# KIT-MBS/pydca

Hardware: AMD Instinct MI355X
Metric: plmDCA L-BFGS iterations/s (L=500 N=50000 q=21) (higher is better)
Workload: dtype f32

## Files before the change

### pydca_amd/csrc/lbfgs_kernels.h

```cpp
#pragma once

#include "dca_internal.h"
#include "plm_plan.h"
#include "vec_kernels.h"

namespace {

template <bool DD> struct DotAcc;
template <> struct DotAcc<false> {
    double hi = 0.0;
    static constexpr double lo = 0.0;
    __device__ __forceinline__ void add(double a, double b) { hi += a * b; }
    __device__ __forceinline__ void wave_reduce() { for (int off = 32; off > 0; off >>= 1) hi += __shfl_down(hi, off); }
};
template <> struct DotAcc<true> {
    double hi = 0.0, lo = 0.0;
    __device__ __forceinline__ void add(double a, double b) { dd_add(hi, lo, __dmul_rn(a, b)); }
    __device__ __forceinline__ void wave_reduce() { dd_wave_reduce(hi, lo); }
};
template <int NV>
__device__ __forceinline__ void dot_block_store(double (*red)[2 * NV], int nv, double* __restrict__ partials, unsigned grid = 0)
{
    __syncthreads();
    if ((int)threadIdx.x < nv) {
// ... 91 lines not shown
        Pack<T> pse; Pack<T> pye;
        _Pragma("unroll") for (int u = 0; u < VEC; ++u) {
            pse.v[u] = px.v[u] - pxp.v[u]; pye.v[u] = pg.v[u] - pgp.v[u];
            acc[0].add((double)pye.v[u], (double)pse.v[u]); acc[1].add((double)pye.v[u], (double)pye.v[u]);
        }
        psk[E] = pse; pyk[E] = pye;
        stp(se, iv, pse); stp(ye, iv, pye);
        _Pragma("unroll") for (int k = 0; k < 5; ++k) {
            _Pragma("unroll") for (int u = 0; u < VEC; ++u) {
                const double gv = pg.v[u]; const double sev = pse.v[u]; const double yev = pye.v[u];
                const double sk = psk[k].v[u]; const double yk = pyk[k].v[u];
                acc[2 + k].add(sk, gv); acc[7 + k].add(yk, gv); acc[12 + k].add(sev, yk); acc[17 + k].add(yev, sk); acc[22 + k].add(yev, yk);
            }
        },
        { const T sev_ = x[i] - xp[i]; const T yev_ = g[i] - gp[i]; se[i] = sev_; ye[i] = yev_;
          const double gv = g[i]; const double sev = sev_; const double yev = yev_;
          acc[0].add(yev, sev); acc[1].add(yev, yev);
          _Pragma("unroll") for (int k = 0; k < 5; ++k) {
              const double sk = k == E ? sev : (double)static_cast<const T*>(P.s[k])[i]; const double yk = k == E ? yev : (double)static_cast<const T*>(P.y[k])[i];
              acc[2 + k].add(sk, gv); acc[7 + k].add(yk, gv); acc[12 + k].add(sev, yk); acc[17 + k].add(yev, sk); acc[22 + k].add(yev, yk);
          } })
    const int lane = threadIdx.x & 63, wv = threadIdx.x >> 6;
#pragma unroll
    for (int v = 0; v < 27; ++v) {
        acc[v].wave_reduce();
        if (lane == 0) { red[wv][2 * v] = acc[v].hi; red[wv][2 * v + 1] = acc[v].lo; }
    }
    dot_block_store<27>(red, 27, partials);
}

template <typename T>
__global__ void vec_compose_kernel(T* __restrict__ d, const T* __restrict__ g, VecPtrs5 P, const DirCoefs* __restrict__ cp, size_t n)
{
    const DirCoefs c = *cp;
    DCA_VEC_LOOP(n, d,
        const Pack<T> pg = ldp(g, iv);
        double v[VEC];
        _Pragma("unroll") for (int u = 0; u < VEC; ++u) v[u] = c.g * (double)pg.v[u];
        _Pragma("unroll") for (int k = 0; k < 5; ++k) {
            const Pack<T> psk = ldp(static_cast<const T*>(P.s[k]), iv); const Pack<T> pyk = ldp(static_cast<const T*>(P.y[k]), iv);
            _Pragma("unroll") for (int u = 0; u < VEC; ++u) v[u] += c.s[k] * (double)psk.v[u] + c.y[k] * (double)pyk.v[u];
        }
        Pack<T> o;
        _Pragma("unroll") for (int u = 0; u < VEC; ++u) o.v[u] = (T)v[u];
        stp(d, iv, o);,
        { double v = c.g * (double)g[i];
          _Pragma("unroll") for (int k = 0; k < 5; ++k)
              v += c.s[k] * (double)static_cast<const T*>(P.s[k])[i] + c.y[k] * (double)static_cast<const T*>(P.y[k])[i];
          d[i] = (T)v; })
}
#undef ldp
#undef stp

__global__ __launch_bounds__(256)
void vec_final_kernel(const double* __restrict__ partials, int nb, int nk, double* __restrict__ out)
{
    __shared__ double redHi[256], redLo[256];
    const int k = blockIdx.x;
    double hi = 0.0, lo = 0.0;
    for (int b = threadIdx.x; b < nb; b += blockDim.x) dd_add2(hi, lo, partials[2 * ((size_t)k * nb + b)], partials[2 * ((size_t)k * nb + b) + 1]);
    dd_block_reduce(hi, lo, redHi, redLo);
    if (threadIdx.x == 0) out[k] = hi + lo;
}

__global__ __launch_bounds__(256)
void dd_sum_chunks_kernel(const double* __restrict__ parts, int n, double* __restrict__ out)
{
    __shared__ double redHi[256], redLo[256];
    const int chunk = (n + gridDim.x - 1) / gridDim.x;
    const int lo_ = blockIdx.x * chunk, hi_ = min(n, lo_ + chunk);
    double hi = 0.0, lo = 0.0;
    for (int b = lo_ + threadIdx.x; b < hi_; b += blockDim.x) dd_add2(hi, lo, parts[2 * (size_t)b], parts[2 * (size_t)b + 1]);
    dd_block_reduce(hi, lo, redHi, redLo);
    if (threadIdx.x == 0) { out[2 * blockIdx.x] = hi; out[2 * blockIdx.x + 1] = lo; }
}
__global__ __launch_bounds__(1024)
void dd_sum_final_kernel(const double* __restrict__ A, int nA, const double* __restrict__ B, int nB, double* __restrict__ out)
{
    __shared__ double redHi[1024], redLo[1024];
    double hi = 0.0, lo = 0.0;
    for (int b = threadIdx.x; b < nA; b += blockDim.x) dd_add2(hi, lo, A[2 * (size_t)b], A[2 * (size_t)b + 1]);
    for (int b = threadIdx.x; b < nB; b += blockDim.x) dd_add2(hi, lo, B[2 * (size_t)b], B[2 * (size_t)b + 1]);
    dd_block_reduce(hi, lo, redHi, redLo);
    if (threadIdx.x == 0) out[0] = hi + lo;
}

template <typename T>
__global__ __launch_bounds__(kVecThreads)
void vec_dot3_fx_kernel(const T* __restrict__ a, const T* __restrict__ b, const T* __restrict__ c, size_t n, double* __restrict__ partials,
                        const double* __restrict__ fxParts, int nFxParts, double* __restrict__ fxChunks)
{
    if (blockIdx.x >= (unsigned)kVecBlocks) {
        __shared__ double redHi[256], redLo[256];
        const int blk = (int)blockIdx.x - kVecBlocks;
        const int chunk = (nFxParts + kSumStageBlocks - 1) / kSumStageBlocks;
        const int lo_ = blk * chunk, hi_ = min(nFxParts, lo_ + chunk);
        double hi = 0.0, lo = 0.0;
        for (int p = lo_ + threadIdx.x; p < hi_; p += blockDim.x) dd_add2(hi, lo, fxParts[2 * (size_t)p], fxParts[2 * (size_t)p + 1]);
        dd_block_reduce(hi, lo, redHi, redLo);
        if (threadIdx.x == 0) { fxChunks[2 * blk] = hi; fxChunks[2 * blk + 1] = lo; }
        return;
    }
    __shared__ double red[kVecThreads / 64][6];
    DotAcc<sizeof(T) == 8> s0, s1, s2;
    DCA_VEC_LOOP_G(n, a, kVecBlocks,
        const Pack<T> pa = ldp_at(a + head_, iv); const Pack<T> pb = ldp_at(b + head_, iv); const Pack<T> pc = ldp_at(c + head_, iv);
// ... 42 lines not shown
```

### pydca_amd/csrc/plm_engine.hip

```cpp
#include <algorithm>
#include <chrono>
#include <cmath>

#include "dca_internal.h"
#include "more_thuente.h"
#include "vec_kernels.h"
#include "plm_plan.h"
#include "plm_stages.h"
#include "lbfgs_kernels.h"

namespace {

static_assert(kPlanXcds == kNumXcd, "the planner deals strips to this many XCDs");

#ifdef DCA_ROUND_ABLATE
__global__ void round_to_f32_kernel(double* __restrict__ p, size_t n)
{
    for (size_t i = blockIdx.x * (size_t)blockDim.x + threadIdx.x; i < n; i += (size_t)gridDim.x * blockDim.x) p[i] = (double)(float)p[i];
}
inline int round_stage_mask() { const char* e = getenv("DCA_ROUND_F32_STAGES"); return e ? atoi(e) : 0; }
#define DCA_ROUND_STAGE(bit, ptr, count)                                                                             \
    do {                                                                                                             \
        if constexpr (sizeof(T) == 8)                                                                                \
            if (round_stage_mask() & (bit))                                                                          \
// ... 1 lines not shown
    } while (0)
#else
#define DCA_ROUND_STAGE(bit, ptr, count) do { } while (0)
#endif

template <typename T>
struct PlmEngine : PlmEngineBase {
    dca_ctx* ctx;
    int N, L, q, Ls;
    double lambda_h = 0, lambda_J = 0;
    int carry_mode = DCA_CARRY_CHUNKED, halo = 0, add_reg = 1;
    bool configured = false;
    PlmPlan plan;
    PlmKnobs knobs;

    T *dx = nullptr, *dg = nullptr, *dxp = nullptr, *dgp = nullptr, *dd = nullptr;
    T* dS[5] = {nullptr, nullptr, nullptr, nullptr, nullptr};
    T* dY[5] = {nullptr, nullptr, nullptr, nullptr, nullptr};
    T *dWt = nullptr, *dSR = nullptr, *dR = nullptr, *dG = nullptr, *dw = nullptr;
    LbfgsDev* dLb = nullptr;
    uint16_t* dXL = nullptr;
    uint16_t* dXT2 = nullptr;
    PairIJ* dPairs = nullptr;
    double *dFxPart = nullptr, *dRegPart = nullptr, *dVecPart = nullptr;
    double *dColPart = nullptr, *dColSum = nullptr;
    double* dColChunk = nullptr;
    bool stripRequested = false, strips = false, stripEmulate = false;
    int sWorld = 1, sRank = 0;
    T *dGrecv = nullptr, *dXsend = nullptr, *dXrecv = nullptr;
    template <typename F> void each_buffer(F f)
    {
        f(dx); f(dg); f(dxp); f(dgp); f(dd);
        for (int i = 0; i < 5; ++i) { f(dS[i]); f(dY[i]); }
        f(dWt); f(dSR); f(dR); f(dG); f(dw); f(dLb); f(dXL); f(dXT2); f(dPairs); f(dFxPart); f(dRegPart); f(dVecPart);
        f(dColPart); f(dColSum); f(dColChunk); f(dGrecv); f(dXsend); f(dXrecv);
    }
    int strip_cs(int r) const { return plm_strip_cs(plan.siteB, q, r); }
    size_t owned_lo(int r) const { return plm_owned_lo(plan.siteB, L, q, r); }
    size_t owned_hi(int r) const { return plm_owned_hi(plan.siteB, L, q, r); }
    bool lbfgs_alloc = false;
    bool deferFx = false, fxPending = false;
    size_t vlo = 0, vn = 0, Ppad = 0;
    dca_comm_hook comm = nullptr;
    void* comm_user = nullptr;
    int comm_rank = 0, comm_world = 0;

    struct {
        bool begun = false, finished = false;
        int status = 0, k = 1, end = 0, iters = 0, evals = 0, max_iterations = 0, verbose = 0;
        double fx = 0, step = 0, xnorm = 0, gnorm = 0, seconds = 0;
        double last_step = 0;
        double dginit = 0;
        bool dginit_on_device = false;
    } o;

    explicit PlmEngine(dca_ctx* c) : ctx(c), N(c->N), L(c->L), q(c->q), Ls(c->Ls) {}

    template <typename U> int dalloc(U** p, size_t n)
    {
        HIP_TRY(dca_dev_malloc(reinterpret_cast<void**>(p), std::max<size_t>(n, 1) * sizeof(U)));
        return DCA_OK;
    }
    void freeall() { each_buffer([](auto*& p) { dca_dev_free(p); p = nullptr; }); }
    ~PlmEngine() override { freeall(); }

    void weights_changed() override { configured = false; o = decltype(o)(); }

    int configure(double lh, double lJ, int cmode, int chunk_, int warm_, int halo_, int add_reg_) override
    {
        if (q != 21 && q != 5) { dca_set_error("plmDCA kernels are built for q = 21 (protein) and q = 5 (RNA); got %d", q); return DCA_ERR_ARG; }
        if (!ctx->have_weights) { dca_set_error("weights must be computed or set before dca_plm_configure"); return DCA_ERR_STATE; }
        if (halo_ < 0 || halo_ >= N) { dca_set_error("halo out of range"); return DCA_ERR_ARG; }
        if (L > 65535) { dca_set_error("L too large"); return DCA_ERR_ARG; }
        configured = false;
        lambda_h = lh; lambda_J = lJ; carry_mode = cmode; halo = halo_; add_reg = add_reg_;
        strips = stripRequested && ctx->comm && ctx->comm_world > 1;
        stripRequested = false;
        sWorld = strips ? ctx->comm_world : 1;
        sRank = strips ? ctx->comm_rank : 0;
#ifdef DCA_ROUND_ABLATE
        stripEmulate = false;
        if (const char* e = getenv("DCA_STRIP_EMULATE")) {
            int er = 0, ew = 1;
            if (sscanf(e, "%d,%d", &er, &ew) == 2 && ew > 1 && er >= 0 && er < ew) { strips = true; stripEmulate = true; sRank = er; sWorld = ew; }
        }
#endif
        if (sWorld > kMaxStripRanks || (strips && sWorld > L)) { dca_set_error("column strips: too many ranks for %d sites", L); return DCA_ERR_ARG; }
        if (strips && (halo || hook || comm)) { dca_set_error("column strips take the whole alignment and no hooks"); return DCA_ERR_ARG; }
        knobs = PlmKnobs::from_env();
        PlmShape shape;
        shape.N = N; shape.L = L; shape.q = q; shape.elemBytes = (int)sizeof(T); shape.halo = halo; shape.chunkArg = chunk_; shape.warmArg = warm_;
        shape.carryMode = carry_mode; shape.stripWorld = sWorld; shape.stripRank = sRank; shape.strips = strips;
        plan = plm_make_plan(shape, knobs, PlmKernelShapes{{logits_seq_per_wg(5), logits_seq_per_wg(21), logits_seq_per_wg(kPairQ)},
                                                           {logits_jt(5), logits_jt(21), logits_jt(kPairQ)}});
        const int Lq = L * q, JT = plan.JT;
        const size_t npairs = (size_t)L * (L - 1) / 2;

        freeall();
        lbfgs_alloc = false;
        o = decltype(o)();

        DCA_TRY(dalloc(&dx, plan.P + kVecPad)); DCA_TRY(dalloc(&dg, plan.P + kVecPad));
        DCA_TRY(dalloc(&dWt, (size_t)plan.Wrows * plan.Cs));
        DCA_TRY(dalloc(&dSR, (size_t)N * plan.Cs));
        DCA_TRY(dalloc(&dR, (size_t)(N + kNC) * plan.Cs));
        HIP_TRY(hipMemsetAsync(dR, 0, (size_t)(N + kNC) * plan.Cs * sizeof(T), ctx->stream));
// ... 59 lines not shown
            hipLaunchKernelGGL(plm_build_pair_states_kernel, dim3(ceil_div(plan.Npad, 256), ceil_div(plan.gUnits, JT) * JT), dim3(256), 0,
                               ctx->stream, ctx->dX, dXL, N, plan.Npad, L, Ls, 0, 0x2000u);
            hipLaunchKernelGGL(plm_build_pair_states_kernel, dim3(ceil_div(plan.NT, 256), plan.gUnits), dim3(256), 0, ctx->stream,
                               ctx->dX, dXT2, N, plan.NT, L, Ls, halo, 0x9000u);
            HIP_TRY(hipGetLastError());
            HIP_TRY(hipStreamSynchronize(ctx->stream));
        } else {
            hipLaunchKernelGGL(plm_build_logit_states_kernel, dim3(ceil_div(plan.Npad, 256), ceil_div(L, JT) * JT), dim3(256), 0,
                               ctx->stream, ctx->dX, dXL, N, plan.Npad, L, Ls);
            hipLaunchKernelGGL(plm_build_states_kernel, dim3(ceil_div(plan.NT, 256), L), dim3(256), 0, ctx->stream,
                               ctx->dX, dXT2, N, L, Ls, halo, plan.NT);
            HIP_TRY(hipGetLastError());
            HIP_TRY(hipStreamSynchronize(ctx->stream));
        }
        configured = true;
        return DCA_OK;
    }

    int configure_strips(double lh, double lJ, int cmode, int chunk_, int warm_) override
    {
        if (!ctx->comm) { dca_set_error("column strips need a communicator: dca_comm_init first"); return DCA_ERR_STATE; }
        if (o.begun && !o.finished) { dca_set_error("the decomposition cannot change during an optimisation"); return DCA_ERR_STATE; }
        const auto hook0 = hook; const auto hookUser0 = hook_user; const auto comm0 = comm; const auto commUser0 = comm_user;
        const int commRank0 = comm_rank, commWorld0 = comm_world;
        hook = nullptr; hook_user = nullptr; comm = nullptr; comm_user = nullptr; comm_rank = comm_world = 0;
        stripRequested = true;
        const int rc = configure(lh, lJ, cmode, chunk_, warm_, 0, 1);
        stripRequested = false;
        if (rc != DCA_OK) { hook = hook0; hook_user = hookUser0; comm = comm0; comm_user = commUser0; comm_rank = commRank0; comm_world = commWorld0; strips = false; }
        return rc;
    }

    int init_x() override
    {
        if (!configured) { dca_set_error("dca_plm_configure first"); return DCA_ERR_STATE; }
        std::vector<T> hw(N);
        HIP_TRY(hipMemcpy(hw.data(), dw, (size_t)N * sizeof(T), hipMemcpyDeviceToHost));
        T meff = 0;
        for (int n = 0; n < N; ++n) meff += hw[n];
        std::vector<T> h((size_t)L * q, (T)0);
        const uint8_t* X = dca_host_msa(ctx);
        if (!X) return DCA_ERR_HIP;
        for (int n = 0; n < N; ++n)
            for (int i = 0; i < L; ++i) h[(size_t)i * q + X[(size_t)n * L + i]] += hw[n];
        for (int i = 0; i < L; ++i) {
            T* hi = h.data() + (size_t)i * q;
            for (int a = 0; a < q; ++a) hi[a] /= meff;
            for (int a = 0; a < q; ++a) hi[a] = std::log(hi[a] * meff + (T)1);
            T s = 0;
            for (int a = 0; a < q; ++a) s += hi[a];
            const T av = s / (T)q;
            for (int a = 0; a < q; ++a) hi[a] -= av;
        }
        HIP_TRY(hipMemsetAsync(dx, 0, plan.P * sizeof(T), ctx->stream));
        HIP_TRY(hipMemcpyAsync(dx, h.data(), h.size() * sizeof(T), hipMemcpyHostToDevice, ctx->stream));
        HIP_TRY(hipStreamSynchronize(ctx->stream));
        return DCA_OK;
    }

    template <typename U> int upload(const U* src, T* dst)
    {
        std::vector<T> tmp(plan.P);
        for (size_t i = 0; i < plan.P; ++i) tmp[i] = (T)src[i];
        HIP_TRY(hipMemcpy(dst, tmp.data(), plan.P * sizeof(T), hipMemcpyHostToDevice));
        return DCA_OK;
    }
    template <typename U> int download(const T* src, U* dst)
    {
        std::vector<T> tmp(plan.P);
        HIP_TRY(hipStreamSynchronize(ctx->stream));
        HIP_TRY(hipMemcpy(tmp.data(), src, plan.P * sizeof(T), hipMemcpyDeviceToHost));
        for (size_t i = 0; i < plan.P; ++i) dst[i] = (U)tmp[i];
        return DCA_OK;
    }
    int set_x(const void* x, int dtype) override
    {
        if (!configured) { dca_set_error("dca_plm_configure first"); return DCA_ERR_STATE; }
        if (dtype == DCA_F32) return upload(static_cast<const float*>(x), dx);
        if (dtype == DCA_F64) return upload(static_cast<const double*>(x), dx);
        return DCA_ERR_ARG;
    }
    int get_x(void* x, int dtype) override
    {
        if (!configured) return DCA_ERR_STATE;
        if (native_mode == 4 && !stripEmulate) DCA_TRY(strip_allgather(dx));
        if (dtype == DCA_F32) return download(dx, static_cast<float*>(x));
        if (dtype == DCA_F64) return download(dx, static_cast<double*>(x));
        return DCA_ERR_ARG;
    }
    int get_g(void* g, int dtype) override
    {
        if (!configured) return DCA_ERR_STATE;
        DCA_TRY(gather_vector(dg));
        if (dtype == DCA_F32) return download(dg, static_cast<float*>(g));
        if (dtype == DCA_F64) return download(dg, static_cast<double*>(g));
        return DCA_ERR_ARG;
    }

    template <int Q> int launch_eval()
    {
        hipStream_t st = ctx->stream;
        const size_t npairs = (size_t)L * (L - 1) / 2;
        {
            ScopedKernelClock kc(ctx, "plm_expand");
            hipLaunchKernelGGL(plm_expand_kernel<T>, dim3((unsigned)npairs), dim3(256), (size_t)q * q * sizeof(T), st,
                               dx, dWt, dPairs, L, q, plan.Cs, plan.cS0, plan.cS1);
        }
        DCA_ROUND_STAGE(1, dWt, (size_t)plan.Wrows * plan.Cs);
        {
            const int numCT = plan.numCT;
            auto launch = [&](auto kern, int QL) -> int {
                const int numNB = plan.Npad / logits_seq_per_wg(QL);
                const int blocks = numCT * numNB;
                const size_t lds = (size_t)2 * 128 * 512 + (size_t)logits_waves(QL) * 256;
                HIP_TRY(hipFuncSetAttribute(reinterpret_cast<const void*>(kern), hipFuncAttributeMaxDynamicSharedMemorySize, (int)lds));
                ScopedKernelClock kc(ctx, "plm_logits");
                hipLaunchKernelGGL(kern, dim3(blocks), dim3(logits_waves(QL) * 64), lds, st, dWt, dXL, dSR, N, plan.Npad, plan.gUnits, plan.Cs, numCT, numNB);
                return DCA_OK;
            };
            bool done = false;
            if constexpr (Q == 5 && sizeof(T) == 4) {
                if (plan.pairs) {
                    if (plan.pairJT == 11) DCA_TRY(launch(plm_logits_kernel<T, kPairQ, 11>, kPairQ));
                    else if (plan.pairJT == 10) DCA_TRY(launch(plm_logits_kernel<T, kPairQ, 10>, kPairQ));
                    else DCA_TRY(launch(plm_logits_kernel<T, kPairQ>, kPairQ));
                    done = true;
                }
            }
            if (!done) DCA_TRY(launch(plm_logits_kernel<T, Q>, Q));
        }
        DCA_ROUND_STAGE(2, dSR, (size_t)N * plan.Cs);
        {
            dim3 grid(ceil_div(plan.Lloc, 64), ceil_div(plan.numScanChunks, 4));
            ScopedKernelClock kc(ctx, "plm_softmax");
            constexpr int softNP = (64 * Q * (int)sizeof(T) + 1023) / 1024;
            const size_t softLds = (size_t)4 * 2 * softNP * 1024;
            HIP_TRY(hipFuncSetAttribute(reinterpret_cast<const void*>(plm_softmax_kernel<T, Q>), hipFuncAttributeMaxDynamicSharedMemorySize, (int)softLds));
            hipLaunchKernelGGL((plm_softmax_kernel<T, Q>), grid, dim3(256), softLds, st, dSR, dR, dx + (size_t)plan.cS0 * q, ctx->dX + plan.cS0, dw, dFxPart,
                               N, plan.Lloc, Ls, plan.Cs, halo, plan.chunk, plan.warm, carry_mode != DCA_CARRY_EXACT ? 1 : 0, plan.numScanChunks, dColChunk);
        }
        DCA_ROUND_STAGE(4, dR, (size_t)N * plan.Cs);
        {
            const size_t lds = (size_t)2 * kNC * kRowBytes;
            const ScatterStage& sc = plan.scatter;
            auto launch = [&](auto kern) -> int {
                HIP_TRY(hipFuncSetAttribute(reinterpret_cast<const void*>(kern), hipFuncAttributeMaxDynamicSharedMemorySize, (int)lds));
                ScopedKernelClock kc(ctx, "plm_scatter");
                for (int i = 0; i < sc.numLaunches; ++i) {
                    const ScatterLaunch& a = sc.launch[i];
                    hipLaunchKernelGGL(kern, dim3(a.gridX, a.gridY), dim3(sc.threads), lds, st, dR, dXT2, dG,
                                       a.N, a.L, a.Cs, a.halo, a.numChunks, a.NT, a.ctBase, a.numPairs, a.splitX, a.numJG, a.chunksPerSplit, a.slabElems, a.blockChunks,
                                       a.firstBlocksX, a.ctBase2, a.numPairs2, a.splitX2, a.chunksPerSplit2);
                }
                if (sc.sumRemCols)
                    hipLaunchKernelGGL(plm_sum_slabs_cols_kernel<T>, dim3(sc.colsGrid), dim3(256), 0, st, dG,
                                       plan.slab_elems(), plan.Cs, sc.col0, sc.ncols, sc.colRows, sc.colSplit, sc.colZero);
// ... 4 lines not shown
                else if (plan.scatWaves == 4) DCA_TRY(launch(plm_scatter_kernel<T, Q, 2, 4>));
                else DCA_TRY(launch(plm_scatter_kernel<T, Q, 2, 16>));
            } else if constexpr (Q == 5) {
                if (plan.pairs) DCA_TRY(launch(plm_scatter_kernel<T, kPairQ, 2, 16>));
                else DCA_TRY(launch(plm_scatter_kernel<T, Q, 2, 16>));
            } else {
                DCA_TRY(launch(plm_scatter_kernel<T, Q, 2, 16>));
            }
        }
        DCA_ROUND_STAGE(8, dG, plan.num_slabs() * plan.slab_elems());
        {
            ScopedKernelClock kc(ctx, "plm_fold");
            const int LqLoc = plan.Lloc * q;
            int foldSlabs = plan.scatSplit;
            if (plan.scatSplit > 2 || (strips && plan.scatSplit > 1)) {
                hipLaunchKernelGGL(plm_sum_slabs_kernel<T>, dim3(2048), dim3(256), 0, st, dG, plan.slab_elems(), plan.scatSplit);
                foldSlabs = 1;
            }
            if (dColSum) {
                if (dColChunk)
                    hipLaunchKernelGGL(plm_colsum_chunks_kernel, dim3(ceil_div(LqLoc, 256), kColSumRowBlocks), dim3(256), 0, st, dColChunk, plan.numScanChunks, LqLoc, dColPart);
                else
                    hipLaunchKernelGGL(plm_colsum_parts_kernel<T>, dim3(ceil_div(LqLoc, 64), kColSumRowBlocks), dim3(256), 0, st, dR, N, plan.Cs, LqLoc, dColPart);
                hipLaunchKernelGGL(plm_colsum_final_kernel, dim3(ceil_div(LqLoc, 256)), dim3(256), 0, st, dColPart, kColSumRowBlocks, LqLoc, dColSum);
            }
            const int nOwned = plan.pairEnd - plan.pairBegin;
            const bool mergeFields = knobs.foldMerge != 0 && !strips && nOwned > 0;
            if (!mergeFields)
            hipLaunchKernelGGL(plm_fold_fields_kernel<T>, dim3(ceil_div(LqLoc, 256)), dim3(256), 0, st, dx + (size_t)plan.cS0 * q, dG, dg + (size_t)plan.cS0 * q,
                               dRegPart + 2 * npairs, LqLoc, q, plan.Cs, (T)lambda_h, add_reg, plan.slab_elems(), foldSlabs, dColSum);
            StripMap sm;
            sm.rank = sRank; sm.world = sWorld; sm.s0 = plan.cS0; sm.s1 = plan.cS1;
            for (int r = 0; r <= sWorld; ++r) sm.site0[r] = plan.siteB[r];
            for (int r = 0; r < sWorld; ++r) { sm.recv[r] = strips && r > sRank ? dGrecv + plan.grecvOff[r] : nullptr; sm.recvCs[r] = strips ? strip_cs(r) : 0; }
            if (strips && !stripEmulate) DCA_TRY(exchange_g());
            const size_t lds = (size_t)kFoldWaves * ((q * q + 3) / 4 * 4) * sizeof(T);
            if (nOwned > 0) {
                const int pairBlocks = ceil_div(nOwned, kFoldWaves);
                FoldFieldsArgs<T> ff{dx + (size_t)plan.cS0 * q, dg + (size_t)plan.cS0 * q, dRegPart + 2 * npairs, LqLoc, (T)lambda_h, dColSum, mergeFields ? pairBlocks : -1};
                hipLaunchKernelGGL(plm_fold_pairs_kernel<T>, dim3((unsigned)(pairBlocks + (mergeFields ? ceil_div(LqLoc, 256) : 0))), dim3(64 * kFoldWaves), lds, st, dx, dG, dg, dPairs,
                                   dRegPart, L, q, plan.Cs, (T)lambda_J, add_reg, plan.slab_elems(), foldSlabs, plan.pairBegin, plan.pairEnd, sm, ff);
            }
        }
        DCA_ROUND_STAGE(16, dg, plan.P);
        fxPending = deferFx;
        if (!deferFx) {
            hipLaunchKernelGGL(dd_sum_chunks_kernel, dim3(kSumStageBlocks), dim3(256), 0, st, dRegPart, plan.nRegPart, dRegPart + 2 * (size_t)plan.nRegPart);
            hipLaunchKernelGGL(dd_sum_final_kernel, dim3(1), dim3(1024), 0, st, dRegPart + 2 * (size_t)plan.nRegPart, kSumStageBlocks, dFxPart, plan.nFxPart, ctx->dScal);
        }
        HIP_TRY(hipGetLastError());
        return DCA_OK;
    }

    int evaluate_async(bool defer_fx = false)
    {
        if (!configured) { dca_set_error("dca_plm_configure first"); return DCA_ERR_STATE; }
        deferFx = defer_fx && knobs.fuseFx != 0 && native_mode == 0 && !hook && !comm && !stripEmulate;
        int rc = (q == 21) ? launch_eval<21>() : launch_eval<5>();
        if (rc != DCA_OK) return rc;
        o.evals += 1;
        if (native_mode == 4) {
        } else if (comm || native_mode == 2 || native_mode == 3) {
            DCA_TRY(do_comm(DCA_COMM_REDUCE_SCATTER, dg, Ppad, (int)sizeof(T) * 8, "reduce-scatter"));
        } else if (native_mode == 1) {
            DCA_TRY(dca_comm_native_reduce(ctx, dg, plan.P, (int)sizeof(T) * 8, ctx->dScal));
        } else if (hook) {
            HIP_TRY(hipStreamSynchronize(ctx->stream));
            if (hook(hook_user, dg, plan.P, (int)sizeof(T) * 8, ctx->dScal) != 0) {
                dca_set_error("reduce hook failed");
                return DCA_ERR_ARG;
            }
        }
        return DCA_OK;
    }

    int do_comm(int op, void* buf, size_t count, int dtype, const char* what)
    {
        if (native_mode >= 2) return dca_comm_native(ctx, op, buf, count, dtype, native_mode == 3);
        HIP_TRY(hipStreamSynchronize(ctx->stream));
        if (comm(comm_user, op, buf, count, dtype) != 0) { dca_set_error("comm hook failed (%s)", what); return DCA_ERR_ARG; }
        return DCA_OK;
    }
    int reduce_scalars(int first, int count)
    {
        if ((!comm && native_mode < 2) || stripEmulate) return DCA_OK;
        return do_comm(DCA_COMM_ALL_REDUCE, ctx->dScal + first, (size_t)count, DCA_F64, "all-reduce");
    }
    int gather_vector(T* v)
    {
        if (!comm && native_mode < 2) return DCA_OK;
        if (native_mode == 4) return stripEmulate ? DCA_OK : strip_allgather(v);
        return do_comm(DCA_COMM_ALL_GATHER, v, Ppad, (int)sizeof(T) * 8, "all-gather");
    }
    int publish_x()
    {
        if (native_mode == 4) return stripEmulate ? DCA_OK : exchange_x();
        return gather_vector(dx);
    }

    int exchange_x()
    {
        const int dt = (int)sizeof(T) * 8;
        const size_t q2 = (size_t)q * q;
        for (int r = sRank + 1; r < sWorld; ++r) {
            const int ni = plan.siteB[r + 1] - plan.siteB[r];
            hipLaunchKernelGGL((strip_pairs_copy_kernel<T, true>), dim3((unsigned)(plan.Lloc * ni)), dim3(64), 0, ctx->stream, dx, dXsend + plan.xsendOff[r], L, q, plan.cS0, plan.cS1, plan.siteB[r], plan.siteB[r + 1]);
        }
        DCA_TRY(dca_comm_p2p_begin(ctx));
        int rc = DCA_OK;
        if (sRank == 0) { for (int r = 1; r < sWorld && rc == DCA_OK; ++r) rc = dca_comm_p2p_send(ctx, dx + (size_t)plan.siteB[r] * q, (size_t)(plan.siteB[r + 1] - plan.siteB[r]) * q, dt, r); }
        else rc = dca_comm_p2p_recv(ctx, dx + (size_t)plan.cS0 * q, (size_t)plan.Lloc * q, dt, 0);
// ... 68 lines not shown
        return DCA_OK;
    }
    int set_vector_sharding(int rank, int world, dca_comm_hook h, void* user) override
    {
        if (!configured) { dca_set_error("dca_plm_configure first"); return DCA_ERR_STATE; }
        if (o.begun && !o.finished) { dca_set_error("vector sharding cannot change during an optimisation"); return DCA_ERR_STATE; }
        if (strips) { dca_set_error("configured for column strips: dca_plm_configure again first"); return DCA_ERR_STATE; }
        if (native_mode >= 2) native_mode = 0;
        if (!h || world < 1) { vlo = 0; vn = plan.P; Ppad = plan.P; comm = nullptr; comm_user = nullptr; comm_rank = comm_world = 0; return DCA_OK; }
        DCA_TRY(set_slices(rank, world));
        comm = h; comm_user = user; comm_rank = rank; comm_world = world;
        return DCA_OK;
    }
    int set_slices(int rank, int world)
    {
        if (rank < 0 || rank >= world || world > 64) { dca_set_error("bad rank / world"); return DCA_ERR_ARG; }
        const size_t slice = (plan.P + (size_t)world * 4 - 1) / ((size_t)world * 4) * 4;
        if (slice * world > plan.P + kVecPad) { dca_set_error("world too large for the vector padding"); return DCA_ERR_ARG; }
        Ppad = slice * world;
        vlo = slice * rank;
        vn = vlo >= plan.P ? 0 : std::min(slice, plan.P - vlo);
        return DCA_OK;
    }
    bool configured_for_comm() const override { return configured; }
    int set_native_comm(int mode) override
    {
        if (!configured) { dca_set_error("dca_plm_configure first"); return DCA_ERR_STATE; }
        if (o.begun && !o.finished) { dca_set_error("the exchange scheme cannot change during an optimisation"); return DCA_ERR_STATE; }
        if (mode != 0 && !ctx->comm) { dca_set_error("no communicator: dca_comm_init first"); return DCA_ERR_STATE; }
        if (mode == 4) { dca_set_error("the column-strip decomposition is set up by dca_plm_configure_strips"); return DCA_ERR_ARG; }
        if (mode < 0 || mode > 3) return DCA_ERR_ARG;
        if (strips) {
            if (mode != 0) { dca_set_error("configured for column strips: dca_plm_configure again first"); return DCA_ERR_STATE; }
            configured = false; strips = false; native_mode = 0; o = decltype(o)();
            return DCA_OK;
        }
        if (mode >= 2) DCA_TRY(set_slices(ctx->comm_rank, ctx->comm_world));
        else { vlo = 0; vn = plan.P; Ppad = plan.P; }
        comm = nullptr; comm_user = nullptr; comm_rank = comm_world = 0;
        if (mode != 0) { hook = nullptr; hook_user = nullptr; }
        native_mode = mode;
        return DCA_OK;
    }

    int read_scalars(int n)
    {
        HIP_TRY(hipMemcpyAsync(ctx->hScal, ctx->dScal, (size_t)n * sizeof(double), hipMemcpyDeviceToHost, ctx->stream));
        HIP_TRY(hipStreamSynchronize(ctx->stream));
        return DCA_OK;
    }

    int gradient(double* fx_out) override
    {
        DCA_TRY(evaluate_async());
        DCA_TRY(reduce_scalars(0, 1));
        DCA_TRY(gather_vector(dg));
        DCA_TRY(read_scalars(1));
        if (fx_out) *fx_out = ctx->hScal[0];
        return DCA_OK;
    }

    void v_neg(T* d, const T* g) { hipLaunchKernelGGL(vec_neg_kernel<T>, dim3(kVecBlocks), dim3(kVecThreads), 0, ctx->stream, d + vlo, g + vlo, vn); }
    void v_step(T* x, const T* xp, double stp, const T* d) { hipLaunchKernelGGL(vec_step_kernel<T>, dim3(kVecBlocks), dim3(kVecThreads), 0, ctx->stream, x + vlo, xp + vlo, (T)stp, d + vlo, vn); }
    int eval_scalars(double* fx, double* gd, double* xx, double* gg)
    {
        if (fxPending) {
            double* const fxChunks = dRegPart + 2 * (size_t)plan.nRegPart;
            hipLaunchKernelGGL(vec_dot3_fx_kernel<T>, dim3(kVecBlocks + kSumStageBlocks), dim3(kVecThreads), 0, ctx->stream, dg + vlo, dd + vlo, dx + vlo, vn, dVecPart,
                               dRegPart, plan.nRegPart, fxChunks);
            hipLaunchKernelGGL(vec_final_fx_kernel, dim3(3 + 1), dim3(1024), 0, ctx->stream, dVecPart, kVecBlocks, 3, ctx->dScal + 1,
                               fxChunks, kSumStageBlocks, dFxPart, plan.nFxPart, ctx->dScal);
            fxPending = false;
        } else {
            hipLaunchKernelGGL(vec_dot3_kernel<T>, dim3(kVecBlocks), dim3(kVecThreads), 0, ctx->stream, dg + vlo, dd + vlo, dx + vlo, vn, dVecPart);
            hipLaunchKernelGGL(vec_final_kernel, dim3(3), dim3(256), 0, ctx->stream, dVecPart, kVecBlocks, 3, ctx->dScal + 1);
        }
        DCA_TRY(reduce_scalars(0, 4));
        DCA_TRY(read_scalars(kSlotDginit + 1));
        *fx = ctx->hScal[0]; *gd = ctx->hScal[1]; *xx = ctx->hScal[2]; *gg = ctx->hScal[3];
        if (o.dginit_on_device) { o.dginit = ctx->hScal[kSlotDginit]; o.dginit_on_device = false; }
        return DCA_OK;
    }

    int lbfgs_begin(int max_iterations, int verbose) override
    {
        if (!configured) { dca_set_error("dca_plm_configure first"); return DCA_ERR_STATE; }
        if (!lbfgs_alloc) {
            DCA_TRY(dalloc(&dxp, plan.P + kVecPad)); DCA_TRY(dalloc(&dgp, plan.P + kVecPad)); DCA_TRY(dalloc(&dd, plan.P + kVecPad));
            for (int i = 0; i < 5; ++i) { DCA_TRY(dalloc(&dS[i], plan.P + kVecPad)); DCA_TRY(dalloc(&dY[i], plan.P + kVecPad)); }
            HIP_TRY(hipMemsetAsync(dxp, 0, (plan.P + kVecPad) * sizeof(T), ctx->stream));
            HIP_TRY(hipMemsetAsync(dgp, 0, (plan.P + kVecPad) * sizeof(T), ctx->stream));
            HIP_TRY(hipMemsetAsync(dd, 0, (plan.P + kVecPad) * sizeof(T), ctx->stream));
            lbfgs_alloc = true;
        }
        for (int i = 0; i < 5; ++i) {
            HIP_TRY(hipMemsetAsync(dS[i], 0, (plan.P + kVecPad) * sizeof(T), ctx->stream));
            HIP_TRY(hipMemsetAsync(dY[i], 0, (plan.P + kVecPad) * sizeof(T), ctx->stream));
        }
        if (!dLb) HIP_TRY(dca_dev_malloc(reinterpret_cast<void**>(&dLb), sizeof(LbfgsDev)));
        HIP_TRY(hipMemsetAsync(dLb, 0, sizeof(LbfgsDev), ctx->stream));
        o = decltype(o)();
        o.max_iterations = max_iterations;
        o.verbose = verbose;
        auto t0 = std::chrono::steady_clock::now();
        DCA_TRY(evaluate_async(true));
        v_neg(dd, dg);
        double fx, gd, xx, gg;
        DCA_TRY(eval_scalars(&fx, &gd, &xx, &gg));
        o.fx = fx;
        o.xnorm = std::sqrt(xx); o.gnorm = std::sqrt(gg);
        const double xn = std::max(o.xnorm, 1.0);
        o.begun = true;
        if (o.gnorm / xn <= 1e-3) { o.status = LB_ALREADY_MINIMIZED; o.finished = true; }
        o.step = 1.0 / std::sqrt(gg);
        o.dginit = -gg;
        o.seconds += std::chrono::duration<double>(std::chrono::steady_clock::now() - t0).count();
        return DCA_OK;
    }

    int line_search(double* stp, double* f, double* xx, double* gg, int* rc_hip)
    {
        const MtParams params{1e-4, 0.9, 1e-16, 1e-20, 1e20, 5};
        const bool deferred = o.dginit_on_device;
        const int ls = mt_line_search(params, stp, f, &o.dginit, deferred, [&](double t, double* ft, double* dgt) {
            v_step(dx, dxp, t, dd);
            DCA_ROUND_STAGE(32, dx, plan.P);
            DCA_TRY(publish_x());
            DCA_TRY(evaluate_async(true));
            return eval_scalars(ft, dgt, xx, gg);
        }, rc_hip);
        if (deferred && ls == LB_INCREASEGRADIENT) o.evals -= 1;
        return ls;
    }

    void lbfgs_end() override { o = decltype(o)(); }
    int lbfgs_iterate(int iterations, dca_plm_stats* st) override
    {
        if (!o.begun) { dca_set_error("dca_plm_lbfgs_begin first"); return DCA_ERR_STATE; }
        auto t0 = std::chrono::steady_clock::now();
        constexpr int M = 5;
        for (int it = 0; it < iterations && !o.finished; ++it) {
            std::swap(dx, dxp);
            std::swap(dg, dgp);
            double xx = 0, gg = 0;
            int rc = 0;
            const int ls = line_search(&o.step, &o.fx, &xx, &gg, &rc);
            if (rc) return rc;
            if (ls < 0) {
                std::swap(dx, dxp);
                std::swap(dg, dgp);
                o.status = ls; o.finished = true;
                break;
            }
            o.xnorm = std::sqrt(xx); o.gnorm = std::sqrt(gg);
            o.iters = o.k;
            o.last_step = o.step;
            if (o.verbose) {
                fprintf(stderr, "Iteration %d:\n", o.k);
                fprintf(stderr, "fx = %f, xnorm = %f, gnorm = %f, step = %f\n\n", o.fx, o.xnorm, o.gnorm, o.step);
            }
            const double xn = std::max(o.xnorm, 1.0);
            if (o.gnorm / xn <= 1e-3) { o.status = 0; o.finished = true; break; }
            if (o.max_iterations != 0 && o.max_iterations < o.k + 1) { o.status = LB_MAXIMUMITERATION; o.finished = true; break; }

            const int e = o.end;
            VecPtrs5 ptrs;
            for (int i = 0; i < M; ++i) { ptrs.s[i] = dS[i] + vlo; ptrs.y[i] = dY[i] + vlo; }
            {
                ScopedKernelClock kc(ctx, "lbfgs_vec");
                auto gram = [&](auto slot) {
                    hipLaunchKernelGGL((vec_diff_gram_kernel<T, decltype(slot)::value>), dim3(kVecBlocks), dim3(kVecThreads), 0, ctx->stream, ptrs, dS[e] + vlo, dY[e] + vlo,
                                       dx + vlo, dxp + vlo, dg + vlo, dgp + vlo, vn, dVecPart);
                };
                switch (e) {
                case 0: gram(std::integral_constant<int, 0>()); break;
                case 1: gram(std::integral_constant<int, 1>()); break;
                case 2: gram(std::integral_constant<int, 2>()); break;
                case 3: gram(std::integral_constant<int, 3>()); break;
                default: gram(std::integral_constant<int, 4>()); break;
                }
                hipLaunchKernelGGL(vec_final_kernel, dim3(27), dim3(256), 0, ctx->stream, dVecPart, kVecBlocks, 27, ctx->dScal + 1);
            }
            DCA_TRY(reduce_scalars(1, 27));
            const int bound = (M <= o.k) ? M : o.k;
            ++o.k;
            o.end = (o.end + 1) % M;
            {
                ScopedKernelClock kc(ctx, "lbfgs_vec");
                hipLaunchKernelGGL(lbfgs_two_loop_kernel, dim3(1), dim3(64), 0, ctx->stream, ctx->dScal, dLb, e, o.end, bound, gg);
                hipLaunchKernelGGL(vec_compose_kernel<T>, dim3(kVecBlocks), dim3(kVecThreads), 0, ctx->stream, dd + vlo, dg + vlo, ptrs, &dLb->cf, vn);
                DCA_ROUND_STAGE(64, dd, plan.P);
                o.dginit_on_device = true;
            }
            o.step = 1.0;
        }
        HIP_TRY(hipStreamSynchronize(ctx->stream));
        o.seconds += std::chrono::duration<double>(std::chrono::steady_clock::now() - t0).count();
        if (st) {
            st->status = o.status; st->iterations = o.iters; st->evaluations = o.evals; st->finished = o.finished ? 1 : 0;
            st->fx = o.fx; st->xnorm = o.xnorm; st->gnorm = o.gnorm; st->step = o.iters ? o.last_step : o.step; st->seconds = o.seconds;
        }
        return DCA_OK;
    }

    int scores(int apc, double* out) override
    {
        if (!configured) return DCA_ERR_STATE;
        if (native_mode == 4 && !stripEmulate) DCA_TRY(strip_allgather(dx));
        const size_t npairs = (size_t)L * (L - 1) / 2;
        double* dOut = nullptr;
        HIP_TRY(dca_dev_malloc(reinterpret_cast<void**>(&dOut), npairs * sizeof(double)));
        int rc = dca_fn_scores(ctx, dx, 0, (int)sizeof(T) * 8, L, q, 0, apc, dOut);
        if (rc == DCA_OK) {
            hipError_t e = hipStreamSynchronize(ctx->stream);
            if (e == hipSuccess) e = hipMemcpy(out, dOut, npairs * sizeof(double), hipMemcpyDeviceToHost);
            if (e != hipSuccess) { dca_set_error("copy scores: %s", hipGetErrorString(e)); rc = DCA_ERR_HIP; }
        }
        dca_dev_free(dOut);
        return rc;
    }
    int pair_couplings(const int* pairs, int npairs, int shift, double* out) override
    {
        if (!configured) return DCA_ERR_STATE;
        if (native_mode == 4 && !stripEmulate) DCA_TRY(strip_allgather(dx));
        return dca_pair_blocks(ctx, dx, 0, (int)sizeof(T) * 8, L, q, 0, pairs, npairs, shift, out);
    }

    int di_scores(const double* reg_fi, int apc, double* out) override
    {
        if (!configured) return DCA_ERR_STATE;
        if (native_mode == 4 && !stripEmulate) DCA_TRY(strip_allgather(dx));
        const size_t npairs = (size_t)L * (L - 1) / 2;
        double *dOut = nullptr, *dFi = nullptr;
        HIP_TRY(dca_dev_malloc(reinterpret_cast<void**>(&dOut), npairs * sizeof(double)));
        if (dca_dev_malloc(reinterpret_cast<void**>(&dFi), (size_t)L * q * sizeof(double)) != hipSuccess) { dca_dev_free(dOut); return DCA_ERR_NOMEM; }
        int rc = DCA_OK;
        if (hipMemcpy(dFi, reg_fi, (size_t)L * q * sizeof(double), hipMemcpyHostToDevice) != hipSuccess) rc = DCA_ERR_HIP;
        if (rc == DCA_OK) rc = dca_di_scores(ctx, dx, 0, (int)sizeof(T) * 8, dFi, L, q, 0, apc, dOut);
        if (rc == DCA_OK) {
            hipError_t e = hipStreamSynchronize(ctx->stream);
            if (e == hipSuccess) e = hipMemcpy(out, dOut, npairs * sizeof(double), hipMemcpyDeviceToHost);
            if (e != hipSuccess) { dca_set_error("copy DI scores: %s", hipGetErrorString(e)); rc = DCA_ERR_HIP; }
        }
        dca_dev_free(dOut); dca_dev_free(dFi);
// ... 12 lines not shown
```

### pydca_amd/csrc/plm_plan.h

```cpp
#pragma once

#include <algorithm>
#include <cstddef>
#include <cstdlib>
#include <vector>

#include "../../include/dca_hip.h"

namespace {

constexpr int kPlanXcds = 8;
constexpr int kPairQ = 25;
constexpr int kNC = 128;
constexpr int kRowBytes = 512;
constexpr int kScatWavesC = 16;
constexpr int kCanonBlock = 16384;
static_assert(kCanonBlock % kNC == 0, "canonical blocks are whole tiles");
constexpr int kColSumRowBlocks = 64;
constexpr int kSumStageBlocks = 64;
constexpr int kMaxStripRanks = 64;
constexpr size_t kVecPad = 256;

struct PlmShape {
    int N = 0, L = 0, q = 0;
    int elemBytes = 4;
    int halo = 0;
    int chunkArg = 0, warmArg = 0;
    int carryMode = DCA_CARRY_CHUNKED;
    int stripWorld = 1, stripRank = 0;
    bool strips = false;
};

struct PlmKnobs {
    int scatterRem = -1;
    int scatterSplit = -1;
    int scatterCanon = -1;
    int scatterWaves = -1;
    int plmPairs = -1;
    int scatterMerge = -1;
    int foldMerge = -1;
    int fuseFx = -1;
    bool is_set(int v) const { return v != -1; }
    static PlmKnobs from_env()
    {
        PlmKnobs k;
        auto rd = [](const char* name, int& v) { if (const char* e = getenv(name)) { v = atoi(e); if (v == -1) v = -2; } };
        rd("DCA_SCATTER_REM", k.scatterRem); rd("DCA_SCATTER_SPLIT", k.scatterSplit); rd("DCA_SCATTER_CANON", k.scatterCanon);
        rd("DCA_SCATTER_WAVES", k.scatterWaves); rd("DCA_PLM_PAIRS", k.plmPairs); rd("DCA_SCATTER_MERGE", k.scatterMerge);
        rd("DCA_FOLD_MERGE", k.foldMerge); rd("DCA_PLM_FUSE_FX", k.fuseFx);
        return k;
    }
};

struct PlmKernelShapes {
    int logitsSeqPerWg[3];
    int logitsJT[3];
    static int slot(int q) { return q == 21 ? 1 : q == kPairQ ? 2 : 0; }
};

struct ScatterLaunch {
    unsigned gridX = 0, gridY = 1;
    int N = 0, L = 0, Cs = 0, halo = 0, numChunks = 0, NT = 0, ctBase = 0, numPairs = 0, splitX = 1, numJG = 0, chunksPerSplit = 0;
    size_t slabElems = 0;
    int blockChunks = 0;
    int firstBlocksX = 0x7fffffff, ctBase2 = 0, numPairs2 = 0, splitX2 = 1, chunksPerSplit2 = 0;
};
struct ScatterStage {
    int threads = 0;
    int numLaunches = 0;
    ScatterLaunch launch[2];
    bool sumRemCols = false;
    unsigned colsGrid = 0;
    int col0 = 0, ncols = 0, colRows = 0, colSplit = 0, colZero = 0;
};

struct PlmPlan {
    std::vector<int> siteB;
    int cS0 = 0, cS1 = 0, Lloc = 0;
    size_t oLo = 0, oHi = 0;
    int pairBegin = 0, pairEnd = 0;
    int chunk = 128, warm = 40, numScanChunks = 0, numScatChunks = 0;
    size_t P = 0;
    int Cs = 0;
    bool pairs = false;
    int gUnits = 0;
    int pairJT = 12;
    int JT = 0;
    int Wrows = 0, Grows = 0, Npad = 0, NT = 0;
    int scatJW = 2, scatWaves = kScatWavesC;
    int scatSplit = 1, scatChunksPerSplit = 0;
    int scatBlockChunks = 0;
    bool scatPerBlock = false;
    int scatRemCT = 0, scatRemSplit = 0, scatRemChunksPerSplit = 0;
    int numCT = 0;
    bool scatDealPairs = false;
    ScatterStage scatter;
    int nFxPart = 0, nRegPart = 0;
    std::vector<size_t> grecvOff, xsendOff, xrecvOff;

    int logits_q(int q) const { return pairs ? kPairQ : q; }
    size_t slab_elems() const { return (size_t)Grows * Cs; }
    int num_slabs() const { return std::max(scatSplit, scatRemSplit); }
// ... 171 lines not shown
```

Measured before the change: 60.27.

## Fuse L-BFGS direction compose, unit trial step and coupling expand into one kernel

Adds a kernel that computes the search direction, writes the trial point x+d at step 1 and scatters the coupling blocks into the expanded W matrix through an LDS tile, all in one launch. The first line-search evaluation at t=1 then skips the separate step and expand kernels. This removes two full passes over the parameter vector and the expand pass over it. The cost is a more complex kernel with an irregular per-row prefix walk and transposed scatter writes, plus state tracking so the precomputed trial is reused only when valid.

Result: faster. 61.63, median of 6 (+2.2%).

```diff
diff --git a/pydca_amd/csrc/lbfgs_kernels.h b/pydca_amd/csrc/lbfgs_kernels.h
--- a/pydca_amd/csrc/lbfgs_kernels.h
+++ b/pydca_amd/csrc/lbfgs_kernels.h
@@ -167,6 +167,124 @@
 #undef ldp
 #undef stp
 
+__host__ __device__ constexpr int fused_step_ti(int q, int elemBytes) { return kRowBytes / elemBytes / q; }
+__host__ __device__ constexpr int fused_step_jc(int q) { return q == 21 ? 4 : 16; }
+constexpr int kFusedStepThreads = 512;
+
+template <typename T>
+__device__ __forceinline__ T compose_elem(const DirCoefs& c, T gv, const T* sv, const T* yv)
+{
+    double v = c.g * (double)gv;
+#pragma unroll
+    for (int k = 0; k < 5; ++k) v += c.s[k] * (double)sv[k] + c.y[k] * (double)yv[k];
+    return (T)v;
+}
+
+template <typename T, int Q>
+__global__ __launch_bounds__(kFusedStepThreads)
+void lbfgs_dir_trial_expand_kernel(T* __restrict__ d, T* __restrict__ xt, T* __restrict__ W, const T* __restrict__ x, const T* __restrict__ g,
+                                   VecPtrs5 P, const DirCoefs* __restrict__ cp, int L, int Cs, int numJC, int pairBlocks)
+{
+    constexpr int VEC = 16 / (int)sizeof(T), TI = fused_step_ti(Q, (int)sizeof(T)), JC = fused_step_jc(Q), Q2 = Q * Q;
+    extern __shared__ __attribute__((aligned(16))) unsigned char dca_smem[];
+    T* tile = reinterpret_cast<T*>(dca_smem);
+    __shared__ size_t sLo[TI];
+    __shared__ int sCnt[TI];
+    __shared__ int sPre[TI + 1];
+    const DirCoefs c = *cp;
+    const T one = (T)1.0;
+    const int tid = threadIdx.x;
+    const int padded = (pairBlocks + 63) / 64 * 64;
+    if ((int)blockIdx.x >= padded) {
+        const size_t e = (size_t)((int)blockIdx.x - padded) * kFusedStepThreads + tid;
+        if (e < (size_t)L * Q) {
+            T sv[5], yv[5];
+#pragma unroll
+            for (int k = 0; k < 5; ++k) { sv[k] = static_cast<const T*>(P.s[k])[e]; yv[k] = static_cast<const T*>(P.y[k])[e]; }
+            const T dv = compose_elem(c, g[e], sv, yv);
+            d[e] = dv;
+            const T v = one * dv;
+            xt[e] = x[e] + v;
+        }
+        return;
+    }
+    const int blk = ((int)blockIdx.x & ~63) | (((int)blockIdx.x & 7) << 3) | (((int)blockIdx.x >> 3) & 7);
+    if (blk >= pairBlocks) return;
+    const int i0 = (blk / numJC) * TI, j0 = (blk % numJC) * JC;
+    const int j1 = min(j0 + JC, L);
+    if (j1 <= i0 + 1) return;
+    if (tid == 0) {
+        int pre = 0;
+        for (int ii = 0; ii < TI; ++ii) {
+            const int i = i0 + ii, jlo = max(j0, i + 1);
+            const int cnt = jlo < j1 ? (j1 - jlo) * Q2 : 0;
+            const size_t before = (size_t)L * (L - 1) / 2 - (size_t)(L - i) * (L - i - 1) / 2;
+            const size_t lo = cnt ? (size_t)L * Q + (before + (size_t)(jlo - i - 1)) * Q2 : 0;
+            sLo[ii] = lo; sCnt[ii] = cnt; sPre[ii] = pre;
+            pre += cnt ? (int)((lo + cnt + VEC - 1) / VEC - lo / VEC) : 0;
+        }
+        sPre[TI] = pre;
+    }
+    __syncthreads();
+    const int total = sPre[TI];
+    for (int idx = tid; idx < total; idx += kFusedStepThreads) {
+        int ii = 0;
+        while (idx >= sPre[ii + 1]) ++ii;
+        const size_t lo = sLo[ii], hi = lo + (size_t)sCnt[ii];
+        const size_t iv = lo / VEC + (size_t)(idx - sPre[ii]);
+        const Pack<T> pg = ldp_at(g, iv); const Pack<T> px = ldp_at(x, iv);
+        Pack<T> psk[5]; Pack<T> pyk[5];
+#pragma unroll
+        for (int k = 0; k < 5; ++k) { psk[k] = ldp_at(static_cast<const T*>(P.s[k]), iv); pyk[k] = ldp_at(static_cast<const T*>(P.y[k]), iv); }
+        Pack<T> od, ox;
+#pragma unroll
+        for (int u = 0; u < VEC; ++u) {
+            T sv[5], yv[5];
+#pragma unroll
+            for (int k = 0; k < 5; ++k) { sv[k] = psk[k].v[u]; yv[k] = pyk[k].v[u]; }
+            od.v[u] = compose_elem(c, pg.v[u], sv, yv);
+            const T v = one * od.v[u];
+            ox.v[u] = px.v[u] + v;
+        }
+        const size_t e0 = iv * VEC;
+        T* const dst = tile + (size_t)(ii * JC + (max(j0, i0 + ii + 1) - j0)) * Q2;
+        if (e0 >= lo && e0 + VEC <= hi) {
+            stp_at(d, iv, od); stp_at(xt, iv, ox);
+#pragma unroll
+            for (int u = 0; u < VEC; ++u) dst[e0 + u - lo] = ox.v[u];
+        } else {
+#pragma unroll
+            for (int u = 0; u < VEC; ++u) {
+                const size_t e = e0 + u;
+                if (e >= lo && e < hi) { d[e] = od.v[u]; xt[e] = ox.v[u]; dst[e - lo] = ox.v[u]; }
+            }
+        }
+    }
+    __syncthreads();
+    {
+        constexpr int WD = JC * Q;
+        int row = tid / WD, col = tid % WD;
+        while (row < TI * Q) {
+            const int ii = row / Q, jj = col / Q;
+            const int i = i0 + ii, j = j0 + jj;
+            if (j > i && j < j1) W[(size_t)(i0 * Q + row) * Cs + j0 * Q + col] = tile[row * Q + ii * ((JC - 1) * Q2) + col + jj * ((Q - 1) * Q)];
+            row += kFusedStepThreads / WD; col += kFusedStepThreads % WD;
+            if (col >= WD) { col -= WD; ++row; }
+        }
+    }
+    {
+        constexpr int WD = TI * Q;
+        int row = tid / WD, col = tid % WD;
+        while (row < JC * Q) {
+            const int jj = row / Q, ii = col / Q;
+            const int i = i0 + ii, j = j0 + jj;
+            if (j > i && j < j1) W[(size_t)(j0 * Q + row) * Cs + i0 * Q + col] = tile[col * Q + ii * ((JC - 1) * Q2) + row + jj * ((Q - 1) * Q)];
+            row += kFusedStepThreads / WD; col += kFusedStepThreads % WD;
+            if (col >= WD) { col -= WD; ++row; }
+        }
+    }
+}
+
 __global__ __launch_bounds__(256)
 void vec_final_kernel(const double* __restrict__ partials, int nb, int nk, double* __restrict__ out)
 {
diff --git a/pydca_amd/csrc/plm_engine.hip b/pydca_amd/csrc/plm_engine.hip
--- a/pydca_amd/csrc/plm_engine.hip
+++ b/pydca_amd/csrc/plm_engine.hip
@@ -77,6 +77,7 @@
         double last_step = 0;
         double dginit = 0;
         bool dginit_on_device = false;
+        bool trial_ready = false;
     } o;
 
     explicit PlmEngine(dca_ctx* c) : ctx(c), N(c->N), L(c->L), q(c->q), Ls(c->Ls) {}
@@ -242,6 +243,7 @@
             const T av = s / (T)q;
             for (int a = 0; a < q; ++a) hi[a] -= av;
         }
+        o.trial_ready = false;
         HIP_TRY(hipMemsetAsync(dx, 0, plan.P * sizeof(T), ctx->stream));
         HIP_TRY(hipMemcpyAsync(dx, h.data(), h.size() * sizeof(T), hipMemcpyHostToDevice, ctx->stream));
         HIP_TRY(hipStreamSynchronize(ctx->stream));
@@ -266,6 +268,7 @@
     int set_x(const void* x, int dtype) override
     {
         if (!configured) { dca_set_error("dca_plm_configure first"); return DCA_ERR_STATE; }
+        o.trial_ready = false;
         if (dtype == DCA_F32) return upload(static_cast<const float*>(x), dx);
         if (dtype == DCA_F64) return upload(static_cast<const double*>(x), dx);
         return DCA_ERR_ARG;
@@ -287,11 +290,11 @@
         return DCA_ERR_ARG;
     }
 
-    template <int Q> int launch_eval()
+    template <int Q> int launch_eval(bool w_ready)
     {
         hipStream_t st = ctx->stream;
         const size_t npairs = (size_t)L * (L - 1) / 2;
-        {
+        if (!w_ready) {
             ScopedKernelClock kc(ctx, "plm_expand");
             hipLaunchKernelGGL(plm_expand_kernel<T>, dim3((unsigned)npairs), dim3(256), (size_t)q * q * sizeof(T), st,
                                dx, dWt, dPairs, L, q, plan.Cs, plan.cS0, plan.cS1);
@@ -402,11 +405,11 @@
         return DCA_OK;
     }
 
-    int evaluate_async(bool defer_fx = false)
+    int evaluate_async(bool defer_fx = false, bool w_ready = false)
     {
         if (!configured) { dca_set_error("dca_plm_configure first"); return DCA_ERR_STATE; }
         deferFx = defer_fx && knobs.fuseFx != 0 && native_mode == 0 && !hook && !comm && !stripEmulate;
-        int rc = (q == 21) ? launch_eval<21>() : launch_eval<5>();
+        int rc = (q == 21) ? launch_eval<21>(w_ready) : launch_eval<5>(w_ready);
         if (rc != DCA_OK) return rc;
         o.evals += 1;
         if (native_mode == 4) {
@@ -581,6 +584,7 @@
 
     int gradient(double* fx_out) override
     {
+        o.trial_ready = false;
         DCA_TRY(evaluate_async());
         DCA_TRY(reduce_scalars(0, 1));
         DCA_TRY(gather_vector(dg));
@@ -651,11 +655,16 @@
     {
         const MtParams params{1e-4, 0.9, 1e-16, 1e-20, 1e20, 5};
         const bool deferred = o.dginit_on_device;
+        bool first = true;
         const int ls = mt_line_search(params, stp, f, &o.dginit, deferred, [&](double t, double* ft, double* dgt) {
-            v_step(dx, dxp, t, dd);
-            DCA_ROUND_STAGE(32, dx, plan.P);
+            const bool ready = o.trial_ready && first && t == 1.0 && fused_step_ok();
+            o.trial_ready = false; first = false;
+            if (!ready) {
+                v_step(dx, dxp, t, dd);
+                DCA_ROUND_STAGE(32, dx, plan.P);
+            }
             DCA_TRY(publish_x());
-            DCA_TRY(evaluate_async(true));
+            DCA_TRY(evaluate_async(true, ready));
             return eval_scalars(ft, dgt, xx, gg);
         }, rc_hip);
         if (deferred && ls == LB_INCREASEGRADIENT) o.evals -= 1;
@@ -663,6 +672,21 @@
     }
 
     void lbfgs_end() override { o = decltype(o)(); }
+    bool fused_step_ok() const
+    {
+#ifdef DCA_ROUND_ABLATE
+        if (round_stage_mask()) return false;
+#endif
+        return knobs.fuseStep != 0 && native_mode == 0 && !hook && !comm && !strips && !stripEmulate && vlo == 0 && vn == plan.P &&
+               plan.cS0 == 0 && plan.cS1 == L;
+    }
+    template <int Q> void launch_fused_step(const VecPtrs5& ptrs)
+    {
+        const int numJC = ceil_div(L, fused_step_jc(Q)), pairBlocks = ceil_div(L, fused_step_ti(Q, (int)sizeof(T))) * numJC;
+        const size_t lds = (size_t)fused_step_ti(Q, (int)sizeof(T)) * fused_step_jc(Q) * Q * Q * sizeof(T);
+        hipLaunchKernelGGL((lbfgs_dir_trial_expand_kernel<T, Q>), dim3((unsigned)(ceil_div(pairBlocks, 64) * 64 + ceil_div(L * Q, kFusedStepThreads))), dim3(kFusedStepThreads), lds,
+                           ctx->stream, dd, dxp, dWt, dx, dg, ptrs, &dLb->cf, L, plan.Cs, numJC, pairBlocks);
+    }
     int lbfgs_iterate(int iterations, dca_plm_stats* st) override
     {
         if (!o.begun) { dca_set_error("dca_plm_lbfgs_begin first"); return DCA_ERR_STATE; }
@@ -678,6 +702,7 @@
             if (ls < 0) {
                 std::swap(dx, dxp);
                 std::swap(dg, dgp);
+                o.trial_ready = false;
                 o.status = ls; o.finished = true;
                 break;
             }
@@ -717,8 +742,13 @@
             {
                 ScopedKernelClock kc(ctx, "lbfgs_vec");
                 hipLaunchKernelGGL(lbfgs_two_loop_kernel, dim3(1), dim3(64), 0, ctx->stream, ctx->dScal, dLb, e, o.end, bound, gg);
-                hipLaunchKernelGGL(vec_compose_kernel<T>, dim3(kVecBlocks), dim3(kVecThreads), 0, ctx->stream, dd + vlo, dg + vlo, ptrs, &dLb->cf, vn);
-                DCA_ROUND_STAGE(64, dd, plan.P);
+                if (fused_step_ok()) {
+                    if (q == 21) launch_fused_step<21>(ptrs); else launch_fused_step<5>(ptrs);
+                    o.trial_ready = true;
+                } else {
+                    hipLaunchKernelGGL(vec_compose_kernel<T>, dim3(kVecBlocks), dim3(kVecThreads), 0, ctx->stream, dd + vlo, dg + vlo, ptrs, &dLb->cf, vn);
+                    DCA_ROUND_STAGE(64, dd, plan.P);
+                }
                 o.dginit_on_device = true;
             }
             o.step = 1.0;
diff --git a/pydca_amd/csrc/plm_plan.h b/pydca_amd/csrc/plm_plan.h
--- a/pydca_amd/csrc/plm_plan.h
+++ b/pydca_amd/csrc/plm_plan.h
@@ -40,6 +40,7 @@
     int scatterMerge = -1;
     int foldMerge = -1;
     int fuseFx = -1;
+    int fuseStep = -1;
     bool is_set(int v) const { return v != -1; }
     static PlmKnobs from_env()
     {
@@ -48,6 +49,7 @@
         rd("DCA_SCATTER_REM", k.scatterRem); rd("DCA_SCATTER_SPLIT", k.scatterSplit); rd("DCA_SCATTER_CANON", k.scatterCanon);
         rd("DCA_SCATTER_WAVES", k.scatterWaves); rd("DCA_PLM_PAIRS", k.plmPairs); rd("DCA_SCATTER_MERGE", k.scatterMerge);
         rd("DCA_FOLD_MERGE", k.foldMerge); rd("DCA_PLM_FUSE_FX", k.fuseFx);
+        rd("DCA_PLM_FUSE_STEP", k.fuseStep);
         return k;
     }
 };
```
